# stella-cv/stella_vslam

Hardware: NVIDIA H100
Metric: frames/sec (ORB+match+local BA) @1920x1080, 2000 kpts (higher is better)
Workload: dtype u8

## Files before the change

stella_vslam_b200/csrc/common.cuh:

```cuda
#pragma once

#include <cuda_runtime.h>

#include <cstdarg>
#include <cstdio>
#include <cstring>
#include <string>

#include <nvtx3/nvToolsExt.h>

#include "../../include/b200vslam.h"

namespace b200 {

void set_error(const char* fmt, ...);
int cuda_fail(cudaError_t e, const char* what, const char* file, int line);

#define B200_CUDA(expr)                                                          \
    do {                                                                         \
        cudaError_t _e = (expr);                                                 \
        if (_e != cudaSuccess) return ::b200::cuda_fail(_e, #expr, __FILE__, __LINE__); \
    } while (0)

template <typename T>
__host__ __device__ constexpr T ceil_div(T a, T b) {
    return (a + b - 1) / b;
}
template <typename T>
__host__ __device__ constexpr T round_up(T a, T b) {
    return ceil_div(a, b) * b;
}

struct NvtxRange {
    explicit NvtxRange(const char* name) { nvtxRangePushA(name); }
    ~NvtxRange() { nvtxRangePop(); }
    NvtxRange(const NvtxRange&) = delete;
    NvtxRange& operator=(const NvtxRange&) = delete;
};
#define B200_CAT2(a, b) a##b
#define B200_CAT(a, b) B200_CAT2(a, b)
#define B200_RANGE(name) ::b200::NvtxRange B200_CAT(b200_nvtx_range_, __LINE__)(name)

int require_device(int device);

struct StagingArena;

namespace lba {
int staging(b200_lba_t h, size_t dev_bytes, size_t host_bytes, cudaStream_t* stream, StagingArena** arena);
}

}
```

stella_vslam_b200/csrc/match_kernels.cu:

```cuda
#include <algorithm>
#include <climits>
#include <cmath>
#include <cstddef>
#include <type_traits>
#include <new>
#include <cstring>
#include <vector>

#include "common.cuh"
#include "essential_ransac.cuh"
#include "staging.cuh"
#include "track_chain.cuh"
#include "triangulate.cuh"

namespace b200 {
namespace match {

constexpr int kTopK = 8;
constexpr int kListRowAlign = 64;
constexpr unsigned kInfKey = 0xFFFFFFFFu;
constexpr unsigned kSentinelIdx = 0x3FFFFFu;
constexpr int kThrLow = 50;
constexpr int kMaxDist = 256;

__device__ __forceinline__ unsigned make_key(unsigned dist, unsigned idx) { return (dist << 22) | idx; }
__device__ __forceinline__ unsigned key_dist(unsigned key) { return key >> 22; }
__device__ __forceinline__ unsigned key_idx(unsigned key) { return key & 0x3FFFFFu; }

__device__ __forceinline__ float angle_diff(float a1, float a2) {
    float ret = __fsub_rn(a1, a2);
    if (ret <= -180.0f) ret = __fadd_rn(ret, 360.0f);
    if (ret > 180.0f) ret = __fsub_rn(ret, 360.0f);
    return ret;
}
__device__ __forceinline__ bool orientation_rejects(float a1, float a2) {
    return fabsf(angle_diff(a1, a2)) > 30.0f;
}

__device__ __forceinline__ unsigned hamming256(const uint4& a0, const uint4& a1, const uint4& b0, const uint4& b1) {
    return __popc(a0.x ^ b0.x) + __popc(a0.y ^ b0.y) + __popc(a0.z ^ b0.z) + __popc(a0.w ^ b0.w) + __popc(a1.x ^ b1.x)
           + __popc(a1.y ^ b1.y) + __popc(a1.z ^ b1.z) + __popc(a1.w ^ b1.w);
}

__global__ void __launch_bounds__(256) hamming_matrix_kernel(const uint4* __restrict__ d1, int n1, const uint4* __restrict__ d2, int n2,
                                                             unsigned short* __restrict__ out) {
    __shared__ uint4 s2[64 * 2];
    const int j0 = blockIdx.x * 64, i = blockIdx.y * blockDim.x + threadIdx.x;
    for (int t = threadIdx.x; t < 128; t += blockDim.x) s2[t] = (j0 + t / 2 < n2) ? d2[(size_t)j0 * 2 + t] : make_uint4(0, 0, 0, 0);
    __syncthreads();
    if (i >= n1) return;
    const uint4 a0 = d1[(size_t)i * 2], a1 = d1[(size_t)i * 2 + 1];
    for (int j = 0; j < 64 && j0 + j < n2; ++j) out[(size_t)i * n2 + j0 + j] = (unsigned short)hamming256(a0, a1, s2[2 * j], s2[2 * j + 1]);
}

struct Side {
    const uint4* desc;
    const unsigned char* angle;
    long long angle_stride;
    const int* off;
    const int* cnt;
};
__device__ __forceinline__ float side_angle(const Side& s, int i) {
    return *reinterpret_cast<const float*>(s.angle + (long long)i * s.angle_stride);
}

constexpr int kTcRows = 128;
constexpr int kTcChunk = 128;
constexpr int kTcThreads = 256;
constexpr int kTcTileBytes = 128 * 256;
struct TcSmem {
    unsigned char a[kTcTileBytes];
    unsigned char b[2][kTcTileBytes];
    uint2 lut[256];
    float ang[2][kTcChunk];
};
__device__ __forceinline__ unsigned long long gmma_desc_k_major(unsigned smem_addr, unsigned lbo_bytes, unsigned sbo_bytes) {
    return (unsigned long long)((smem_addr >> 4) & 0x3FFFu) | ((unsigned long long)((lbo_bytes >> 4) & 0x3FFFu) << 16)
           | ((unsigned long long)((sbo_bytes >> 4) & 0x3FFFu) << 32);
}
__device__ __forceinline__ void wgmma_s8_m64n128k32(unsigned (&d)[64], unsigned long long da, unsigned long long db, unsigned accumulate) {
    asm volatile(
        "{\n\t.reg .pred p;\n\t"
        "setp.ne.b32 p, %66, 0;\n\t"
        "wgmma.mma_async.sync.aligned.m64n128k32.s32.s8.s8 {%0, %1, %2, %3, %4, %5, %6, %7, %8, %9, %10, %11, %12, %13, %14, %15, %16, %17, "
        "%18, %19, %20, %21, %22, %23, %24, %25, %26, %27, %28, %29, %30, %31, %32, %33, %34, %35, %36, %37, %38, %39, %40, %41, %42, %43, %44, "
        "%45, %46, %47, %48, %49, %50, %51, %52, %53, %54, %55, %56, %57, %58, %59, %60, %61, %62, %63}, %64, %65, p;\n\t}"
        : "+r"(d[0]), "+r"(d[1]), "+r"(d[2]), "+r"(d[3]), "+r"(d[4]), "+r"(d[5]), "+r"(d[6]), "+r"(d[7]), "+r"(d[8]), "+r"(d[9]), "+r"(d[10]),
          "+r"(d[11]), "+r"(d[12]), "+r"(d[13]), "+r"(d[14]), "+r"(d[15]), "+r"(d[16]), "+r"(d[17]), "+r"(d[18]), "+r"(d[19]), "+r"(d[20]),
          "+r"(d[21]), "+r"(d[22]), "+r"(d[23]), "+r"(d[24]), "+r"(d[25]), "+r"(d[26]), "+r"(d[27]), "+r"(d[28]), "+r"(d[29]), "+r"(d[30]),
          "+r"(d[31]), "+r"(d[32]), "+r"(d[33]), "+r"(d[34]), "+r"(d[35]), "+r"(d[36]), "+r"(d[37]), "+r"(d[38]), "+r"(d[39]), "+r"(d[40]),
          "+r"(d[41]), "+r"(d[42]), "+r"(d[43]), "+r"(d[44]), "+r"(d[45]), "+r"(d[46]), "+r"(d[47]), "+r"(d[48]), "+r"(d[49]), "+r"(d[50]),
          "+r"(d[51]), "+r"(d[52]), "+r"(d[53]), "+r"(d[54]), "+r"(d[55]), "+r"(d[56]), "+r"(d[57]), "+r"(d[58]), "+r"(d[59]), "+r"(d[60]),
          "+r"(d[61]), "+r"(d[62]), "+r"(d[63])
        : "l"(da), "l"(db), "r"(accumulate)
        : "memory");
}
__device__ __forceinline__ void wgmma_fence_operands(unsigned (&d)[64]) {
#pragma unroll
    for (int i = 0; i < 64; ++i) asm volatile("" : "+r"(d[i])::"memory");
}
__device__ __forceinline__ void tc_expand_half(unsigned char* tile, const uint2* lut, int r, int c0, uint4 bits) {
    unsigned char* dst = tile + (r >> 3) * 128 + (r & 7) * 16;
    const unsigned w[4] = {bits.x, bits.y, bits.z, bits.w};
#pragma unroll
    for (int i = 0; i < 8; ++i) {
        const unsigned hw = (w[i >> 1] >> (16 * (i & 1))) & 0xFFFFu;
        const uint2 lo = lut[hw & 0xFFu], hi = lut[hw >> 8];
        *reinterpret_cast<uint4*>(dst + (c0 + i) * 2048) = make_uint4(lo.x, lo.y, hi.x, hi.y);
    }
}
__device__ __forceinline__ void tc_zero_half(unsigned char* tile, int r, int c0) {
    unsigned char* dst = tile + (r >> 3) * 128 + (r & 7) * 16;
#pragma unroll
    for (int i = 0; i < 8; ++i) *reinterpret_cast<uint4*>(dst + (c0 + i) * 2048) = make_uint4(0, 0, 0, 0);
}
__device__ __forceinline__ void insert_key(unsigned (&top)[kTopK], unsigned key) {
    top[kTopK - 1] = key;
#pragma unroll
    for (int k = kTopK - 1; k > 0; --k) {
        if (top[k] < top[k - 1]) {
            const unsigned t = top[k];
            top[k] = top[k - 1];
            top[k - 1] = t;
        }
    }
}

__global__ void __launch_bounds__(kTcThreads, 2) topk_tc_kernel(Side S1, Side S2, const unsigned char* __restrict__ valid2, int check_orientation,
                                                                unsigned* __restrict__ lists, int list_rows, unsigned cap) {
    extern __shared__ __align__(1024) unsigned char tc_smem_raw[];
    TcSmem& sm = *reinterpret_cast<TcSmem*>(tc_smem_raw);
    const uint4* __restrict__ desc1 = S1.desc;
    const uint4* __restrict__ desc2 = S2.desc;
    const int p = blockIdx.y;
    const int b1 = S1.off[p], n1 = S1.cnt[p];
    const int b2 = S2.off[p], n2 = S2.cnt[p];
    const int row0 = blockIdx.x * kTcRows;
    if (row0 >= n2) return;
    const int tid = threadIdx.x, lane = tid & 31;
    for (int e = tid; e < 256; e += kTcThreads) {
        unsigned lo = 0, hi = 0;
#pragma unroll
        for (int i = 0; i < 4; ++i) {
            lo |= (((e >> i) & 1) ? 0x01u : 0xFFu) << (8 * i);
            hi |= (((e >> (4 + i)) & 1) ? 0x01u : 0xFFu) << (8 * i);
        }
        sm.lut[e] = make_uint2(lo, hi);
    }
    __syncthreads();
    const int rtid = tid & 127, half = tid >> 7;
    if (row0 + rtid < n2) tc_expand_half(sm.a, sm.lut, rtid, 8 * half, desc2[(size_t)(b2 + row0 + rtid) * 2 + half]);
    else tc_zero_half(sm.a, rtid, 8 * half);
    const int r_lo = 64 * half + 16 * ((tid >> 5) & 3) + (lane >> 2);
    bool active[2];
    float qa[2];
    unsigned thr[2], top[2][kTopK];
#pragma unroll
    for (int h = 0; h < 2; ++h) {
        const int row = row0 + r_lo + 8 * h;
        active[h] = row < n2 && (!valid2 || valid2[b2 + row]);
        qa[h] = active[h] ? side_angle(S2, b2 + row) : 0.f;
        thr[h] = active[h] ? make_key(cap + 1u, 0u) : 0u;
#pragma unroll
        for (int k = 0; k < kTopK; ++k) top[h][k] = kInfKey;
    }
    const unsigned a_addr = (unsigned)__cvta_generic_to_shared(sm.a) + (unsigned)(half * 8 * 128);
    const unsigned b_addr[2] = {(unsigned)__cvta_generic_to_shared(sm.b[0]), (unsigned)__cvta_generic_to_shared(sm.b[1])};
    const int n_chunks = (n1 + kTcChunk - 1) / kTcChunk;
    uint4 nb = make_uint4(0, 0, 0, 0);
    float nang = 0.f;
    auto fetch = [&](int j) {
        if (j < n1) {
            nb = desc1[(size_t)(b1 + j) * 2 + half];
            if (half == 0) nang = side_angle(S1, b1 + j);
        }
    };
    auto stage = [&](int c) {
        const int j = c * kTcChunk + rtid;
        if (j < n1) {
            tc_expand_half(sm.b[c & 1], sm.lut, rtid, 8 * half, nb);
            if (half == 0) sm.ang[c & 1][rtid] = nang;
        } else {
            tc_zero_half(sm.b[c & 1], rtid, 8 * half);
        }
        fetch(j + kTcChunk);
    };
    fetch(rtid);
    if (n_chunks > 0) stage(0);
    asm volatile("fence.proxy.async.shared::cta;" ::: "memory");
    __syncthreads();
    unsigned acc[64];
#pragma unroll
    for (int i = 0; i < 64; ++i) acc[i] = 0u;
    for (int c = 0; c < n_chunks; ++c) {
        const int buf = c & 1, c0 = c * kTcChunk;
        wgmma_fence_operands(acc);
        asm volatile("wgmma.fence.sync.aligned;" ::: "memory");
#pragma unroll
        for (int ks = 0; ks < 8; ++ks)
            wgmma_s8_m64n128k32(acc, gmma_desc_k_major(a_addr + ks * 4096, 2048, 128), gmma_desc_k_major(b_addr[buf] + ks * 4096, 2048, 128),
                                ks > 0 ? 1u : 0u);
        asm volatile("wgmma.commit_group.sync.aligned;" ::: "memory");
        if (c + 1 < n_chunks) {
            stage(c + 1);
            asm volatile("fence.proxy.async.shared::cta;" ::: "memory");
        }
        asm volatile("wgmma.wait_group.sync.aligned 0;" ::: "memory");
        wgmma_fence_operands(acc);
        const unsigned kbase = (256u << 21) + (unsigned)c0;
        auto scan = [&](auto full_chunk) {
#pragma unroll
            for (int i = 0; i < kTcChunk / 8; ++i) {
                const int col = 8 * i + 2 * (lane & 3);
                unsigned key[2][2];
#pragma unroll
                for (int h = 0; h < 2; ++h)
#pragma unroll
                    for (int u = 0; u < 2; ++u) {
                        key[h][u] = (unsigned)((int)acc[4 * i + 2 * h + u] * -(1 << 21)) + (kbase + (unsigned)(col + u));
                        if (!decltype(full_chunk)::value && c0 + col + u >= n1) key[h][u] = kInfKey;
                    }
                const bool hit = min(key[0][0], key[0][1]) < thr[0] || min(key[1][0], key[1][1]) < thr[1];
                if (__any_sync(0xFFFFFFFFu, hit)) {
#pragma unroll
                    for (int h = 0; h < 2; ++h)
#pragma unroll
                        for (int u = 0; u < 2; ++u) {
                            if (key[h][u] < thr[h]) {
                                if (check_orientation && orientation_rejects(sm.ang[buf][col + u], qa[h])) continue;
                                insert_key(top[h], key[h][u]);
                                thr[h] = min(thr[h], top[h][kTopK - 1]);
                            }
                        }
                }
            }
        };
        if (c0 + kTcChunk <= n1) scan(std::true_type{});
        else scan(std::false_type{});
        __syncthreads();
    }
    unsigned* park = reinterpret_cast<unsigned*>(sm.b[0]);
#pragma unroll
    for (int h = 0; h < 2; ++h)
#pragma unroll
        for (int k = 0; k < kTopK; ++k) park[((r_lo + 8 * h) * 4 + (lane & 3)) * kTopK + k] = top[h][k];
    __syncthreads();
    if (tid < kTcRows) {
        unsigned t[kTopK];
#pragma unroll
        for (int k = 0; k < kTopK; ++k) t[k] = park[tid * 4 * kTopK + k];
        for (int q = 1; q < 4; ++q) {
#pragma unroll
            for (int k2 = 0; k2 < kTopK; ++k2) {
                const unsigned key = park[(tid * 4 + q) * kTopK + k2];
                if (key < t[kTopK - 1]) insert_key(t, key);
            }
        }
#pragma unroll
        for (int k = 0; k < kTopK; ++k)
            if (t[k] == kInfKey && cap < (unsigned)kMaxDist) t[k] = make_key(cap + 1u, kSentinelIdx);
        if (row0 + tid < n2) {
            unsigned* o = lists + ((size_t)p * list_rows + row0 + tid) * kTopK;
#pragma unroll
            for (int k = 0; k < kTopK; ++k) o[k] = t[k];
        }
    }
}

__device__ __forceinline__ unsigned warp_min(unsigned v) {
#pragma unroll
    for (int s = 16; s > 0; s >>= 1) v = min(v, __shfl_xor_sync(0xFFFFFFFFu, v, s));
    return v;
}

__device__ void exact_row(const uint4* desc1, const unsigned char* angle1, long long angle_stride, int n1, const volatile unsigned* taken,
                          uint4 q0, uint4 q1, float qa, int check_orientation, int lane, unsigned* best_key, unsigned* second_dist) {
    unsigned k1 = kInfKey, k2 = kInfKey;
    for (int i0 = lane; i0 < n1; i0 += 128) {
        uint4 a0[4], a1[4];
        float ang[4];
#pragma unroll
        for (int u = 0; u < 4; ++u) {
            const int i = min(i0 + 32 * u, n1 - 1);
            a0[u] = desc1[(size_t)i * 2];
            a1[u] = desc1[(size_t)i * 2 + 1];
            ang[u] = *reinterpret_cast<const float*>(angle1 + (long long)i * angle_stride);
        }
#pragma unroll
        for (int u = 0; u < 4; ++u) {
            const int i = i0 + 32 * u;
            if (i >= n1) continue;
            if ((taken[i >> 5] >> (i & 31)) & 1u) continue;
            if (check_orientation && orientation_rejects(ang[u], qa)) continue;
            const unsigned key = make_key(hamming256(q0, q1, a0[u], a1[u]), (unsigned)i);
            if (key < k1) {
                k2 = k1;
                k1 = key;
            } else if (key < k2) {
                k2 = key;
            }
        }
    }
    const unsigned b = warp_min(k1);
    const unsigned mine = (k1 == b) ? k2 : k1;
    const unsigned s = warp_min(mine);
    *best_key = b;
    *second_dist = (s == kInfKey) ? (unsigned)kMaxDist : key_dist(s);
}

__device__ __forceinline__ int decide_row(const unsigned (&keys)[kTopK], bool full, unsigned tail_dist, const volatile unsigned* taken, float lowe_ratio,
                                          unsigned* best) {
    unsigned best_key = kInfKey, second_dist = kMaxDist;
    int n_live = 0;
#pragma unroll
    for (int k = 0; k < kTopK; ++k) {
        const unsigned key = keys[k];
        if (key == kInfKey) continue;
        const unsigned i1 = key_idx(key);
        if ((taken[i1 >> 5] >> (i1 & 31)) & 1u) continue;
// ... 1115 lines not shown
        if (!s_removed) continue;
        ++n_removed;
        for (int i = tid; i < K.n; i += kCullThreads) {
            const int l = K.kp_lm[i];
            if (l < 0 || __ldcg(P.live_count + l) == 0) continue;
            const int j = cull_own_obs(P, P.off[l], P.off[l + 1], r);
            P.erased[j] = 1;
            atomicSub(P.live_weight + l, (int)P.weight[j]);
            atomicSub(P.live_count + l, 1);
        }
        __syncthreads();
    }
    if (tid == 0) *P.n_removed = n_removed;
}

struct ChainTimer {
    cudaEvent_t ev[7] = {};
    bool timed = false;
    int create() {
        for (cudaEvent_t& e : ev)
            if (!e) B200_CUDA(cudaEventCreate(&e));
        return B200_OK;
    }
    int elapsed(int stage, float* ms) const {
        if (!ms || stage < 0 || stage > 6 || !timed) return B200_ERR_INVALID;
        B200_CUDA(cudaEventElapsedTime(ms, ev[stage == 6 ? 0 : stage], ev[stage == 6 ? 6 : stage + 1]));
        return B200_OK;
    }
    void destroy() {
        for (cudaEvent_t e : ev)
            if (e) cudaEventDestroy(e);
    }
};
enum ChainId { kLocalMapChain, kMotionChain, kRobustChain, kBowChain, kChains };

struct Matcher {
    int device = 0;
    cudaStream_t own_stream = nullptr, stream = nullptr;
    cudaStream_t side_stream = nullptr;
    cudaEvent_t ev_topk = nullptr, ev_resolved = nullptr;
    bool async_resolve = false, resolve_pending = false;
    bool timing = false;
    cudaEvent_t ev_t[3] = {nullptr, nullptr, nullptr};
    ChainTimer chain_timers[kChains];
    int join() {
        if (resolve_pending) {
            B200_CUDA(cudaStreamWaitEvent(stream, ev_resolved, 0));
            resolve_pending = false;
        }
        return B200_OK;
    }
    unsigned* d_lists = nullptr;
    size_t lists_cap = 0;
    int* d_matched = nullptr;
    size_t matched_cap = 0;
    unsigned* d_taken = nullptr;
    size_t taken_cap = 0;
    StagingArena arena;

    int grow(void** p, size_t* cap, size_t bytes) {
        if (bytes <= *cap) return B200_OK;
        B200_CUDA(cudaStreamSynchronize(stream));
        if (*p) B200_CUDA(cudaFree(*p));
        *p = nullptr;
        *cap = 0;
        const size_t want = bytes + bytes / 4 + 256;
        B200_CUDA(cudaMalloc(p, want));
        *cap = want;
        return B200_OK;
    }

    int run(cudaStream_t st, int n_problems, const Side& S1, const Side& S2, const void* valid2, int max_n1, int max_n2, float lowe, int check_ori,
            void* pairs, int pairs_stride, void* n_pairs, bool device_call = false) {
        if (n_problems <= 0) return B200_OK;
        if (max_n1 >= (1 << 22) - 1) {
            set_error("brute-force matcher supports < 4194304 keypoints per frame");
            return B200_ERR_INVALID;
        }
        int rc;
        if ((rc = join())) return rc;
        max_n1 = std::max(max_n1, 1);
        if (pairs_stride < max_n1) {
            set_error("pairs_stride %d is smaller than the largest frame (%d keypoints)", pairs_stride, max_n1);
            return B200_ERR_CAPACITY;
        }
        const int taken_words = ceil_div(max_n1, 32);
        const int list_rows = std::max(1, ceil_div(max_n2, kListRowAlign)) * kListRowAlign;
        if ((rc = grow((void**)&d_lists, &lists_cap, sizeof(unsigned) * kTopK * (size_t)list_rows * n_problems))) return rc;
        if ((rc = grow((void**)&d_matched, &matched_cap, sizeof(int) * (size_t)max_n1 * n_problems))) return rc;
        if ((rc = grow((void**)&d_taken, &taken_cap, sizeof(unsigned) * (size_t)taken_words * n_problems))) return rc;
        if (timing) B200_CUDA(cudaEventRecord(ev_t[0], st));
        const float need = lowe > 0.f ? std::ceil((float)kThrLow / lowe) + 1.f : (float)kMaxDist;
        const unsigned cap = (unsigned)std::min((float)kMaxDist, std::max((float)kThrLow, need));
        B200_CUDA(cudaFuncSetAttribute(topk_tc_kernel, cudaFuncAttributeMaxDynamicSharedMemorySize, (int)sizeof(TcSmem) + 1024));
        topk_tc_kernel<<<dim3(ceil_div(std::max(max_n2, 1), kTcRows), n_problems), kTcThreads, sizeof(TcSmem) + 1024, st>>>(
            S1, S2, (const unsigned char*)valid2, check_ori, d_lists, list_rows, cap);
        if (timing) B200_CUDA(cudaEventRecord(ev_t[1], st));
        const size_t state_bytes = sizeof(unsigned) * ((size_t)taken_words + 2 * (size_t)max_n1);
        const size_t stage_bytes = sizeof(unsigned) * 9 * (size_t)max_n1;
        const int use_smem = (state_bytes + stage_bytes <= 200 * 1024) ? 2 : (state_bytes <= 200 * 1024 ? 1 : 0);
        const size_t rs_bytes = use_smem == 2 ? state_bytes + stage_bytes : state_bytes;
        if (use_smem && rs_bytes > 48 * 1024)
            B200_CUDA(cudaFuncSetAttribute(resolve_kernel, cudaFuncAttributeMaxDynamicSharedMemorySize, (int)rs_bytes));
        cudaStream_t rs = st;
        if (async_resolve && device_call) {
            B200_CUDA(cudaEventRecord(ev_topk, st));
            B200_CUDA(cudaStreamWaitEvent(side_stream, ev_topk, 0));
            rs = side_stream;
        }
        resolve_kernel<<<n_problems, 32, use_smem ? rs_bytes : 0, rs>>>(S1, S2, (const unsigned char*)valid2, d_lists, lowe, check_ori, d_matched,
                                                                        d_taken, taken_words, list_rows, max_n1, pairs_stride, (int*)pairs,
                                                                        (int*)n_pairs, use_smem);
        B200_CUDA(cudaGetLastError());
        if (timing) B200_CUDA(cudaEventRecord(ev_t[2], rs));
        if (rs != st) {
            B200_CUDA(cudaEventRecord(ev_resolved, side_stream));
            resolve_pending = true;
        }
        return B200_OK;
    }
};

template <class Dev = GuidedDev>
static int guided_resolve_smem(const char* who, int n, size_t* bytes) {
    *bytes = (size_t)std::max(n, 1) * 6 + 16;
    if (*bytes > 200 * 1024) {
        set_error("%s: %d keypoints per frame exceed the on-chip occupancy table", who, n);
        return B200_ERR_CAPACITY;
    }
    if (*bytes > 48 * 1024)
        B200_CUDA(cudaFuncSetAttribute(guided_resolve_kernel<Dev>, cudaFuncAttributeMaxDynamicSharedMemorySize, (int)*bytes));
    return B200_OK;
}

}
}

struct b200_matcher_s {
    b200::match::Matcher m;
};

namespace b200 {
namespace chain {
using match::GuidedDev;

static bool search_params_valid(const b200_track_params_t& p) {
    return p.grid_cols > 0 && p.grid_rows > 0 && (long long)p.grid_cols * p.grid_rows <= (1 << 20) && p.img_bounds[1] > p.img_bounds[0]
           && p.img_bounds[3] > p.img_bounds[2] && p.max_candidates >= 0;
}
// ... 245 lines not shown
    sh.k4 = p.cam.k4; sh.distortion = p.cam.distortion;
    sh.cols = p.cam.cols; sh.rows = p.cam.rows;
    sh.fxb = p.focal_x_baseline;
    sh.min_x = p.img_bounds[0]; sh.max_x = p.img_bounds[1]; sh.min_y = p.img_bounds[2]; sh.max_y = p.img_bounds[3];
    sh.ray_cos_thr = p.ray_cos_thr;
    sh.log_scale_factor = p.log_scale_factor;
    sh.margin = p.margin;
    sh.delta = p.monocular ? std::sqrt(5.99146f) : std::sqrt(7.81473f);
    sh.num_levels = p.num_levels;
    for (unsigned l = 0; l < 32; ++l) {
        sh.scale_factors[l] = p.scale_factors[std::min(l, p.num_levels - 1)];
        sh.inv_level_sigma_sq[l] = p.inv_level_sigma_sq[std::min(l, p.num_levels - 1)];
    }
    sh.monocular = p.monocular ? 1 : 0;
    sh.true_baseline = true_baseline;
    return sh;
}
}
}

using b200::match::Side;

extern "C" {

int b200_matcher_create(int device, b200_matcher_t* out) {
    if (!out) return B200_ERR_INVALID;
    int rc = b200::require_device(device);
    if (rc) return rc;
    b200_matcher_s* h = new (std::nothrow) b200_matcher_s();
    if (!h) return B200_ERR_INVALID;
    h->m.device = device;
    cudaError_t e = cudaStreamCreateWithFlags(&h->m.own_stream, cudaStreamNonBlocking);
    if (e == cudaSuccess) e = cudaStreamCreateWithFlags(&h->m.side_stream, cudaStreamNonBlocking);
    if (e == cudaSuccess) e = cudaEventCreateWithFlags(&h->m.ev_topk, cudaEventDisableTiming);
    if (e == cudaSuccess) e = cudaEventCreateWithFlags(&h->m.ev_resolved, cudaEventDisableTiming);
    for (int i = 0; i < 3 && e == cudaSuccess; ++i) e = cudaEventCreate(&h->m.ev_t[i]);
    if (e != cudaSuccess) {
        delete h;
        return b200::cuda_fail(e, "stream creation", __FILE__, __LINE__);
    }
    h->m.stream = h->m.own_stream;
    *out = h;
    return B200_OK;
}

int b200_matcher_destroy(b200_matcher_t h) {
    if (!h) return B200_OK;
    cudaSetDevice(h->m.device);
    cudaStreamSynchronize(h->m.stream);
    if (h->m.side_stream) cudaStreamSynchronize(h->m.side_stream);
    cudaFree(h->m.d_lists);
    cudaFree(h->m.d_matched);
    cudaFree(h->m.d_taken);
    h->m.arena.release();
    for (int i = 0; i < 3; ++i)
        if (h->m.ev_t[i]) cudaEventDestroy(h->m.ev_t[i]);
    for (b200::match::ChainTimer& t : h->m.chain_timers) t.destroy();
    if (h->m.ev_topk) cudaEventDestroy(h->m.ev_topk);
    if (h->m.ev_resolved) cudaEventDestroy(h->m.ev_resolved);
    if (h->m.side_stream) cudaStreamDestroy(h->m.side_stream);
    if (h->m.own_stream) cudaStreamDestroy(h->m.own_stream);
    delete h;
    return B200_OK;
}

int b200_matcher_set_async_resolve(b200_matcher_t h, int enable) {
    if (!h) return B200_ERR_INVALID;
    int rc = h->m.join();
    if (rc) return rc;
    h->m.async_resolve = enable != 0;
    return B200_OK;
}

int b200_matcher_enable_timing(b200_matcher_t h, int enable) {
    if (!h) return B200_ERR_INVALID;
    h->m.timing = enable != 0;
    return B200_OK;
}

int b200_matcher_stage_ms(b200_matcher_t h, int stage, float* ms) {
    if (!h || !ms || stage < 0 || stage > 1) return B200_ERR_INVALID;
    B200_CUDA(cudaEventSynchronize(h->m.ev_t[stage + 1]));
    B200_CUDA(cudaEventElapsedTime(ms, h->m.ev_t[stage], h->m.ev_t[stage + 1]));
    return B200_OK;
}

int b200_matcher_join(b200_matcher_t h) {
    if (!h) return B200_ERR_INVALID;
    return h->m.join();
}

int b200_matcher_set_stream(b200_matcher_t h, void* stream, int use_own) {
    if (!h) return B200_ERR_INVALID;
    B200_CUDA(cudaStreamSynchronize(h->m.stream));
    if (h->m.side_stream) B200_CUDA(cudaStreamSynchronize(h->m.side_stream));
    h->m.resolve_pending = false;
    h->m.stream = use_own ? h->m.own_stream : (cudaStream_t)stream;
    return B200_OK;
}

int b200_matcher_sync(b200_matcher_t h) {
    if (!h) return B200_ERR_INVALID;
    if (h->m.resolve_pending) {
        B200_CUDA(cudaStreamSynchronize(h->m.side_stream));
        h->m.resolve_pending = false;
    }
// ... 1404 lines not shown
    B200_CUDA(cudaGetLastError());
    B200_CUDA(A.download(in_bytes, out_end, st));
    B200_CUDA(cudaStreamSynchronize(st));
    for (int p = 0; p < n_problems; ++p) {
        b200_cull_problem_t& P = problems[p];
        const int* o = A.host<const int>(lay[p].out);
        P.n_removed = o[0];
        for (int r = 0; r < P.n_covisibilities; ++r) {
            b200_cull_keyframe_t& K = P.covisibilities[r];
            K.n_valid = o[1 + 4 * r];
            K.n_redundant = o[2 + 4 * r];
            K.skipped = o[3 + 4 * r];
            K.removed = o[4 + 4 * r];
        }
        P.status = B200_OK;
    }
    return B200_OK;
}

int b200_match_cross_check(const int32_t* idx2_in_1, int n1, const int32_t* idx1_in_2, int n2, int32_t* mutual_out, int32_t* n_mutual) {
    if (n1 < 0 || n2 < 0 || (n1 > 0 && (!idx2_in_1 || !mutual_out)) || (n2 > 0 && !idx1_in_2)) return B200_ERR_INVALID;
    int n = 0;
    for (int i = 0; i < n1; ++i) {
        const int j = idx2_in_1[i];
        const bool keep = 0 <= j && j < n2 && idx1_in_2[j] == i;
        mutual_out[i] = keep ? j : -1;
        n += keep;
    }
    if (n_mutual) *n_mutual = n;
    return B200_OK;
}

int b200_hamming_matrix(b200_matcher_t h, const uint8_t* desc1, int n1, const uint8_t* desc2, int n2, uint16_t* dist) {
    if (!h || n1 < 0 || n2 < 0) return B200_ERR_INVALID;
    if (n1 == 0 || n2 == 0) return B200_OK;
    if (!desc1 || !desc2 || !dist) return B200_ERR_INVALID;
    auto& m = h->m;
    B200_CUDA(cudaSetDevice(m.device));
    b200::Layout L;
    const size_t o_d1 = L.take((size_t)32 * n1), o_d2 = L.take((size_t)32 * n2), o_out = L.take<uint16_t>((size_t)n1 * n2);
    int rc = m.arena.reserve(L.end, 0, m.stream);
    if (rc) return rc;
    unsigned char* s = m.arena.d;
    B200_CUDA(cudaMemcpyAsync(s + o_d1, desc1, (size_t)32 * n1, cudaMemcpyHostToDevice, m.stream));
    B200_CUDA(cudaMemcpyAsync(s + o_d2, desc2, (size_t)32 * n2, cudaMemcpyHostToDevice, m.stream));
    b200::match::hamming_matrix_kernel<<<dim3(b200::ceil_div(n2, 64), b200::ceil_div(n1, 256)), 256, 0, m.stream>>>(
        (const uint4*)(s + o_d1), n1, (const uint4*)(s + o_d2), n2, (unsigned short*)(s + o_out));
    B200_CUDA(cudaGetLastError());
    B200_CUDA(cudaMemcpyAsync(dist, s + o_out, sizeof(uint16_t) * (size_t)n1 * n2, cudaMemcpyDeviceToHost, m.stream));
    B200_CUDA(cudaStreamSynchronize(m.stream));
    return B200_OK;
}

}

namespace b200 {
namespace mapping {

using match::PairsDev;
using tri::TriKfDev;

struct TriProblemDev {
    int k1, k2;
    float cos_thr, ratio_factor;
    int begin;
};

__global__ void __launch_bounds__(256) triangulate_pairs_kernel(const TriKfDev* __restrict__ kfs, const TriProblemDev* __restrict__ ps, int n_problems,
                                                                int total, const int2* __restrict__ matches, double* __restrict__ pos_w,
                                                                unsigned char* __restrict__ ok, int* __restrict__ unconverged) {
    const int t = blockIdx.x * blockDim.x + threadIdx.x;
    if (t >= total) return;
    int lo = 0, hi = n_problems - 1;
    while (lo < hi) {
        const int mid = (lo + hi + 1) >> 1;
        if (ps[mid].begin <= t) lo = mid;
        else hi = mid - 1;
    }
    const TriProblemDev& P = ps[lo];
    const int2 m = matches[t];
    double p[3];
    const int r = tri::two_view_triangulate(kfs[P.k1], kfs[P.k2], m.x, m.y, P.cos_thr, P.ratio_factor, p);
    if (r < 0) atomicAdd(unconverged, 1);
    pos_w[3 * (size_t)t] = p[0];
    pos_w[3 * (size_t)t + 1] = p[1];
    pos_w[3 * (size_t)t + 2] = p[2];
    ok[t] = r == 1;
}

struct ChainKfDev {
    int cur;
    int n_nb;
    int nb_begin;
    int* n_created_rank;
    int* n_created;
    int* created_rank;
    int2* created_idx;
    double* created_pos;
};

constexpr int kClaimThreads = 256;

__global__ void __launch_bounds__(kClaimThreads) landmark_claim_kernel(const TriKfDev* __restrict__ kfs, const float2* __restrict__ nb_consts, const ChainKfDev* __restrict__ ks,
                                                                       const PairsDev* __restrict__ pairs, int n_kf, int rank,
                                                                       int* __restrict__ unconverged) {
    __shared__ int warp_total[kClaimThreads / 32];
// ... 451 lines not shown
```

stella_vslam_b200/csrc/orb_kernels.cu:

```cuda
#include <cuda.h>

#include <algorithm>
#include <cmath>
#include <new>
#include <vector>

#include "camera_model.cuh"
#include "common.cuh"
#include "staging.cuh"
#include "track_chain.cuh"
#include "util_trig.cuh"

namespace b200 {
namespace orb {

constexpr int kMaxLevels = 16;
constexpr int kBorder = 19;
constexpr int kCell = 64;
constexpr int kOverlap = 6;
constexpr int kTileMax = kCell + kOverlap;
constexpr int kTilePitch = 80;

struct LevelGeom {
    int w, h, pitch;
    unsigned long long offset;
    float sf;
    int nx, ny;
    double delta_x, delta_y;
    int grid_base;
    int ncols;
    float size;
    int tab_x, tab_y;
};

struct Geom {
    int num_levels;
    int grid_cells;
    int ini_thr, min_thr;
    LevelGeom lv[kMaxLevels];
};

struct CellDesc {
    unsigned short level, i, j, min_x, min_y, w, h, pad;
};

struct RawKp {
    short x, y;
    unsigned char m;
    unsigned char level;
    unsigned short pad;
};

struct ResizeTap {
    short ofs, w0, w1, pad;
};

struct Images {
    const unsigned char* img0;
    unsigned long long pitch0, fstride0;
    unsigned char* pyr;
    unsigned long long pyr_fstride;
};

__device__ __forceinline__ const unsigned char* level_ptr(const Images& im, const Geom& g, int level, int frame, int* pitch) {
    if (level == 0) {
        *pitch = (int)im.pitch0;
        return im.img0 + (size_t)frame * im.fstride0;
    }
    *pitch = g.lv[level].pitch;
    return im.pyr + (size_t)frame * im.pyr_fstride + g.lv[level].offset;
}

struct TmapSet {
    CUtensorMap m[kMaxLevels];
};

__device__ __forceinline__ unsigned smem_u32(const void* p) { return (unsigned)__cvta_generic_to_shared(p); }

__device__ __forceinline__ void mbar_init(unsigned long long* bar, unsigned count) {
    asm volatile("mbarrier.init.shared::cta.b64 [%0], %1;" ::"r"(smem_u32(bar)), "r"(count));
    asm volatile("fence.mbarrier_init.release.cluster;" ::: "memory");
}
__device__ __forceinline__ void mbar_expect_tx(unsigned long long* bar, unsigned bytes) {
    asm volatile("mbarrier.arrive.expect_tx.shared::cta.b64 _, [%0], %1;" ::"r"(smem_u32(bar)), "r"(bytes) : "memory");
}
__device__ __forceinline__ void mbar_wait(unsigned long long* bar, unsigned parity) {
    asm volatile(
        "{\n\t.reg .pred p;\n\t"
        "WAIT_%=:\n\t"
        "mbarrier.try_wait.parity.shared::cta.b64 p, [%0], %1;\n\t"
        "@p bra DONE_%=;\n\t"
        "bra WAIT_%=;\n\t"
        "DONE_%=:\n\t}" ::"r"(smem_u32(bar)),
        "r"(parity)
        : "memory");
}
__device__ __forceinline__ void tma_load_3d(void* smem_dst, const CUtensorMap* tmap, int x, int y, int z, unsigned long long* bar) {
    asm volatile("cp.async.bulk.tensor.3d.shared::cluster.global.mbarrier::complete_tx::bytes [%0], [%1, {%2, %3, %4}], [%5];" ::"r"(
                     smem_u32(smem_dst)),
                 "l"(reinterpret_cast<unsigned long long>(tmap)), "r"(x), "r"(y), "r"(z), "r"(smem_u32(bar))
                 : "memory");
}

constexpr int kRzRows = 8;

__global__ void __launch_bounds__(128) resize_kernel(const __grid_constant__ Geom g, Images im, const ResizeTap* __restrict__ taps, int level) {
    const LevelGeom& L = g.lv[level];
    const int frame = blockIdx.z;
    int spitch;
    const unsigned char* src = level_ptr(im, g, level - 1, frame, &spitch);
    unsigned char* dst = im.pyr + (size_t)frame * im.pyr_fstride + L.offset;
    const int sw = g.lv[level - 1].w, sh = g.lv[level - 1].h;
    const int dxq = (blockIdx.x * blockDim.x + threadIdx.x) * 4;
    const int dy0 = blockIdx.y * kRzRows;
    if (dxq >= L.pitch) return;
    const int n_valid = min(4, L.w - dxq);
    const unsigned store_mask = n_valid >= 4 ? 0xFFFFFFFFu : (n_valid <= 0 ? 0u : ((1u << (8 * n_valid)) - 1u));
    int ofs[4], ofs1[4];
    unsigned w01[4];
#pragma unroll
    for (int k = 0; k < 4; ++k) {
        const ResizeTap t = taps[L.tab_x + min(dxq + k, L.w - 1)];
        ofs[k] = t.ofs;
        ofs1[k] = min((int)t.ofs + 1, sw - 1);
        w01[k] = ((unsigned)t.w0 & 0xFFFFu) | ((unsigned)t.w1 << 16);
    }
    int rowA = -1, rowB = -1;
    unsigned hA[4] = {0, 0, 0, 0}, hB[4] = {0, 0, 0, 0};
    auto hrow = [&](int sy, unsigned (&h)[4]) {
        const unsigned char* r = src + (size_t)sy * spitch;
#pragma unroll
        for (int k = 0; k < 4; ++k) h[k] = __dp2a_lo(w01[k], (unsigned)r[ofs[k]] | ((unsigned)r[ofs1[k]] << 8), 0u) >> 4;
    };
    const int dy_end = min(dy0 + kRzRows, L.h);
    unsigned char* drow = dst + (size_t)dy0 * L.pitch + dxq;
    for (int dy = dy0; dy < dy_end; ++dy, drow += L.pitch) {
        const ResizeTap ty = taps[L.tab_y + dy];
        const int s0 = min(max((int)ty.ofs, 0), sh - 1), s1 = min(max((int)ty.ofs + 1, 0), sh - 1);
        if (s0 != rowA) {
            if (s0 == rowB) {
#pragma unroll
                for (int k = 0; k < 4; ++k) hA[k] = hB[k];
            } else {
                hrow(s0, hA);
            }
            rowA = s0;
        }
        if (s1 != rowB) {
            if (s1 == rowA) {
// ... 1958 lines not shown
```

Before: 10260.

## Pre-expand B descriptors once and stream them via bulk-async copies in top-k

Adds a separate kernel that expands each problem's S1 descriptors into the ±1 int8 tile layout (plus angles) once in global memory. The top-k tensor-core kernel then loads these pre-expanded chunks with mbarrier-tracked bulk async copies into a double-buffered ring, so expansion is no longer repeated by every row block. Orientation gating moves into the branch-free scan, and a warp-quad threshold tightening runs after each chunk. This costs extra global memory and bandwidth for the expanded tiles (about 32KB per 128 descriptors) plus one more kernel launch, and adds optional phase-profiling instrumentation.

```diff
diff --git a/stella_vslam_b200/csrc/common.cuh b/stella_vslam_b200/csrc/common.cuh
--- a/stella_vslam_b200/csrc/common.cuh
+++ b/stella_vslam_b200/csrc/common.cuh
@@ -45,6 +45,27 @@
 
 struct StagingArena;
 
+__device__ __forceinline__ unsigned smem_u32(const void* p) { return (unsigned)__cvta_generic_to_shared(p); }
+
+__device__ __forceinline__ void mbar_init(unsigned long long* bar, unsigned count) {
+    asm volatile("mbarrier.init.shared::cta.b64 [%0], %1;" ::"r"(smem_u32(bar)), "r"(count));
+    asm volatile("fence.mbarrier_init.release.cluster;" ::: "memory");
+}
+__device__ __forceinline__ void mbar_expect_tx(unsigned long long* bar, unsigned bytes) {
+    asm volatile("mbarrier.arrive.expect_tx.shared::cta.b64 _, [%0], %1;" ::"r"(smem_u32(bar)), "r"(bytes) : "memory");
+}
+__device__ __forceinline__ void mbar_wait(unsigned long long* bar, unsigned parity) {
+    asm volatile(
+        "{\n\t.reg .pred p;\n\t"
+        "WAIT_%=:\n\t"
+        "mbarrier.try_wait.parity.shared::cta.b64 p, [%0], %1;\n\t"
+        "@p bra DONE_%=;\n\t"
+        "bra WAIT_%=;\n\t"
+        "DONE_%=:\n\t}" ::"r"(smem_u32(bar)),
+        "r"(parity)
+        : "memory");
+}
+
 namespace lba {
 int staging(b200_lba_t h, size_t dev_bytes, size_t host_bytes, cudaStream_t* stream, StagingArena** arena);
 }
diff --git a/stella_vslam_b200/csrc/match_kernels.cu b/stella_vslam_b200/csrc/match_kernels.cu
--- a/stella_vslam_b200/csrc/match_kernels.cu
+++ b/stella_vslam_b200/csrc/match_kernels.cu
@@ -68,11 +68,17 @@
 constexpr int kTcChunk = 128;
 constexpr int kTcThreads = 256;
 constexpr int kTcTileBytes = 128 * 256;
+struct TcChunk {
+    unsigned char b[kTcTileBytes];
+    float ang[kTcChunk];
+};
+constexpr int kTcChunkBytes = (int)sizeof(TcChunk);
+static_assert(kTcChunkBytes % 128 == 0, "B tiles of the ring stay 128-byte aligned");
 struct TcSmem {
     unsigned char a[kTcTileBytes];
-    unsigned char b[2][kTcTileBytes];
+    TcChunk chunk[2];
     uint2 lut[256];
-    float ang[2][kTcChunk];
+    unsigned long long full[2];
 };
 __device__ __forceinline__ unsigned long long gmma_desc_k_major(unsigned smem_addr, unsigned lbo_bytes, unsigned sbo_bytes) {
     return (unsigned long long)((smem_addr >> 4) & 0x3FFFu) | ((unsigned long long)((lbo_bytes >> 4) & 0x3FFFu) << 16)
@@ -109,6 +115,15 @@
         *reinterpret_cast<uint4*>(dst + (c0 + i) * 2048) = make_uint4(lo.x, lo.y, hi.x, hi.y);
     }
 }
+__device__ __forceinline__ uint2 tc_lut_entry(int e) {
+    unsigned lo = 0, hi = 0;
+#pragma unroll
+    for (int i = 0; i < 4; ++i) {
+        lo |= (((e >> i) & 1) ? 0x01u : 0xFFu) << (8 * i);
+        hi |= (((e >> (4 + i)) & 1) ? 0x01u : 0xFFu) << (8 * i);
+    }
+    return make_uint2(lo, hi);
+}
 __device__ __forceinline__ void tc_zero_half(unsigned char* tile, int r, int c0) {
     unsigned char* dst = tile + (r >> 3) * 128 + (r & 7) * 16;
 #pragma unroll
@@ -126,28 +141,58 @@
     }
 }
 
-__global__ void __launch_bounds__(kTcThreads, 2) topk_tc_kernel(Side S1, Side S2, const unsigned char* __restrict__ valid2, int check_orientation,
+#ifdef B200_TOPK_PHASES
+enum { kPhWarpChunks, kPhIssueStage, kPhWait, kPhScan, kPhInsert, kPhHits, kPhInserts, kPhSync, kPhMerge, kPhRows, kPhGated, kPhCount };
+constexpr int kPhHistBins = 66;
+__device__ unsigned long long g_topk_phase[kPhCount + kPhHistBins];
+#define TOPK_PH(...) __VA_ARGS__
+#else
+#define TOPK_PH(...)
+#endif
+
+__global__ void __launch_bounds__(256) topk_expand_kernel(Side S1, unsigned char* __restrict__ bexp, int chunk_stride) {
+    __shared__ uint2 lut[256];
+    const int p = blockIdx.y, c = blockIdx.x;
+    const int b1 = S1.off[p], n1 = S1.cnt[p];
+    if (c * kTcChunk >= n1) return;
+    const int tid = threadIdx.x, r = tid & 127, half = tid >> 7, j = c * kTcChunk + r;
+    lut[tid] = tc_lut_entry(tid);
+    __syncthreads();
+    TcChunk* dst = reinterpret_cast<TcChunk*>(bexp + ((size_t)p * chunk_stride + c) * kTcChunkBytes);
+    if (j < n1) tc_expand_half(dst->b, lut, r, 8 * half, S1.desc[(size_t)(b1 + j) * 2 + half]);
+    else tc_zero_half(dst->b, r, 8 * half);
+    if (half == 0) dst->ang[r] = j < n1 ? side_angle(S1, b1 + j) : 0.f;
+}
+
+__global__ void __launch_bounds__(kTcThreads, 2) topk_tc_kernel(Side S1, Side S2, const unsigned char* __restrict__ bexp, int chunk_stride,
+                                                                const unsigned char* __restrict__ valid2, int check_orientation,
                                                                 unsigned* __restrict__ lists, int list_rows, unsigned cap) {
     extern __shared__ __align__(1024) unsigned char tc_smem_raw[];
     TcSmem& sm = *reinterpret_cast<TcSmem*>(tc_smem_raw);
-    const uint4* __restrict__ desc1 = S1.desc;
     const uint4* __restrict__ desc2 = S2.desc;
     const int p = blockIdx.y;
-    const int b1 = S1.off[p], n1 = S1.cnt[p];
+    const int n1 = S1.cnt[p];
     const int b2 = S2.off[p], n2 = S2.cnt[p];
     const int row0 = blockIdx.x * kTcRows;
     if (row0 >= n2) return;
     const int tid = threadIdx.x, lane = tid & 31;
-    for (int e = tid; e < 256; e += kTcThreads) {
-        unsigned lo = 0, hi = 0;
-#pragma unroll
-        for (int i = 0; i < 4; ++i) {
-            lo |= (((e >> i) & 1) ? 0x01u : 0xFFu) << (8 * i);
-            hi |= (((e >> (4 + i)) & 1) ? 0x01u : 0xFFu) << (8 * i);
-        }
-        sm.lut[e] = make_uint2(lo, hi);
+    for (int e = tid; e < 256; e += kTcThreads) sm.lut[e] = tc_lut_entry(e);
+    if (tid == 0) {
+        mbar_init(&sm.full[0], 1);
+        mbar_init(&sm.full[1], 1);
     }
     __syncthreads();
+    const int n_chunks = min((n1 + kTcChunk - 1) / kTcChunk, chunk_stride);
+    const unsigned char* bsrc = bexp + (size_t)p * chunk_stride * kTcChunkBytes;
+    auto load = [&](int c) {
+        unsigned long long* bar = &sm.full[c & 1];
+        mbar_expect_tx(bar, (unsigned)kTcChunkBytes);
+        asm volatile("cp.async.bulk.shared::cluster.global.mbarrier::complete_tx::bytes [%0], [%1], %2, [%3];" ::"r"(smem_u32(&sm.chunk[c & 1])),
+                     "l"(bsrc + (size_t)c * kTcChunkBytes), "r"((unsigned)kTcChunkBytes), "r"(smem_u32(bar))
+                     : "memory");
+    };
+    if (tid == 0)
+        for (int c = 0; c < min(2, n_chunks); ++c) load(c);
     const int rtid = tid & 127, half = tid >> 7;
     if (row0 + rtid < n2) tc_expand_half(sm.a, sm.lut, rtid, 8 * half, desc2[(size_t)(b2 + row0 + rtid) * 2 + half]);
     else tc_zero_half(sm.a, rtid, 8 * half);
@@ -165,35 +210,17 @@
         for (int k = 0; k < kTopK; ++k) top[h][k] = kInfKey;
     }
     const unsigned a_addr = (unsigned)__cvta_generic_to_shared(sm.a) + (unsigned)(half * 8 * 128);
-    const unsigned b_addr[2] = {(unsigned)__cvta_generic_to_shared(sm.b[0]), (unsigned)__cvta_generic_to_shared(sm.b[1])};
-    const int n_chunks = (n1 + kTcChunk - 1) / kTcChunk;
-    uint4 nb = make_uint4(0, 0, 0, 0);
-    float nang = 0.f;
-    auto fetch = [&](int j) {
-        if (j < n1) {
-            nb = desc1[(size_t)(b1 + j) * 2 + half];
-            if (half == 0) nang = side_angle(S1, b1 + j);
-        }
-    };
-    auto stage = [&](int c) {
-        const int j = c * kTcChunk + rtid;
-        if (j < n1) {
-            tc_expand_half(sm.b[c & 1], sm.lut, rtid, 8 * half, nb);
-            if (half == 0) sm.ang[c & 1][rtid] = nang;
-        } else {
-            tc_zero_half(sm.b[c & 1], rtid, 8 * half);
-        }
-        fetch(j + kTcChunk);
-    };
-    fetch(rtid);
-    if (n_chunks > 0) stage(0);
+    const unsigned b_addr[2] = {smem_u32(sm.chunk[0].b), smem_u32(sm.chunk[1].b)};
     asm volatile("fence.proxy.async.shared::cta;" ::: "memory");
     __syncthreads();
     unsigned acc[64];
 #pragma unroll
     for (int i = 0; i < 64; ++i) acc[i] = 0u;
+    TOPK_PH(unsigned long long ph[kPhCount] = {}; unsigned n_pass[2] = {0u, 0u}, n_gated[2] = {0u, 0u}; long long t0 = clock64(); long long t1 = t0;)
     for (int c = 0; c < n_chunks; ++c) {
         const int buf = c & 1, c0 = c * kTcChunk;
+        TOPK_PH(t0 = clock64(); ph[kPhWarpChunks] += 1;)
+        mbar_wait(&sm.full[buf], (unsigned)(c >> 1) & 1u);
         wgmma_fence_operands(acc);
         asm volatile("wgmma.fence.sync.aligned;" ::: "memory");
 #pragma unroll
@@ -201,17 +228,16 @@
             wgmma_s8_m64n128k32(acc, gmma_desc_k_major(a_addr + ks * 4096, 2048, 128), gmma_desc_k_major(b_addr[buf] + ks * 4096, 2048, 128),
                                 ks > 0 ? 1u : 0u);
         asm volatile("wgmma.commit_group.sync.aligned;" ::: "memory");
-        if (c + 1 < n_chunks) {
-            stage(c + 1);
-            asm volatile("fence.proxy.async.shared::cta;" ::: "memory");
-        }
+        TOPK_PH(t1 = clock64(); ph[kPhIssueStage] += t1 - t0; t0 = t1;)
         asm volatile("wgmma.wait_group.sync.aligned 0;" ::: "memory");
         wgmma_fence_operands(acc);
+        TOPK_PH(t1 = clock64(); ph[kPhWait] += t1 - t0; t0 = t1;)
         const unsigned kbase = (256u << 21) + (unsigned)c0;
-        auto scan = [&](auto full_chunk) {
+        auto scan = [&](auto full_chunk, auto gate) {
 #pragma unroll
             for (int i = 0; i < kTcChunk / 8; ++i) {
                 const int col = 8 * i + 2 * (lane & 3);
+                const float2 ang = decltype(gate)::value ? *reinterpret_cast<const float2*>(&sm.chunk[buf].ang[col]) : make_float2(0.f, 0.f);
                 unsigned key[2][2];
 #pragma unroll
                 for (int h = 0; h < 2; ++h)
@@ -219,27 +245,48 @@
                     for (int u = 0; u < 2; ++u) {
                         key[h][u] = (unsigned)((int)acc[4 * i + 2 * h + u] * -(1 << 21)) + (kbase + (unsigned)(col + u));
                         if (!decltype(full_chunk)::value && c0 + col + u >= n1) key[h][u] = kInfKey;
+                        TOPK_PH(n_pass[h] += active[h] && key[h][u] < make_key(cap + 1u, 0u);)
+                        if (decltype(gate)::value && orientation_rejects(u ? ang.y : ang.x, qa[h])) key[h][u] = kInfKey;
+                        TOPK_PH(n_gated[h] += active[h] && key[h][u] < make_key(cap + 1u, 0u);)
                     }
                 const bool hit = min(key[0][0], key[0][1]) < thr[0] || min(key[1][0], key[1][1]) < thr[1];
                 if (__any_sync(0xFFFFFFFFu, hit)) {
+                    TOPK_PH(const long long ti = clock64(); ph[kPhHits] += 1;)
 #pragma unroll
                     for (int h = 0; h < 2; ++h)
 #pragma unroll
                         for (int u = 0; u < 2; ++u) {
                             if (key[h][u] < thr[h]) {
-                                if (check_orientation && orientation_rejects(sm.ang[buf][col + u], qa[h])) continue;
                                 insert_key(top[h], key[h][u]);
                                 thr[h] = min(thr[h], top[h][kTopK - 1]);
+                                TOPK_PH(ph[kPhInserts] += 1;)
                             }
                         }
+                    TOPK_PH(ph[kPhInsert] += clock64() - ti;)
                 }
             }
         };
-        if (c0 + kTcChunk <= n1) scan(std::true_type{});
-        else scan(std::false_type{});
+        const bool full = c0 + kTcChunk <= n1;
+        if (check_orientation) full ? scan(std::true_type{}, std::true_type{}) : scan(std::false_type{}, std::true_type{});
+        else full ? scan(std::true_type{}, std::false_type{}) : scan(std::false_type{}, std::false_type{});
+#pragma unroll
+        for (int h = 0; h < 2; ++h) {
+            unsigned b7 = min(top[h][7], __shfl_xor_sync(0xFFFFFFFFu, top[h][7], 1));
+            b7 = min(b7, __shfl_xor_sync(0xFFFFFFFFu, b7, 2));
+            unsigned b1 = max(top[h][1], __shfl_xor_sync(0xFFFFFFFFu, top[h][1], 1));
+            b1 = max(b1, __shfl_xor_sync(0xFFFFFFFFu, b1, 2));
+            const unsigned o3 = __shfl_xor_sync(0xFFFFFFFFu, top[h][3], 1);
+            const unsigned lo = min(top[h][3], o3), hi = max(top[h][3], o3);
+            const unsigned b3 = min(max(lo, __shfl_xor_sync(0xFFFFFFFFu, lo, 2)), min(hi, __shfl_xor_sync(0xFFFFFFFFu, hi, 2)));
+            thr[h] = min(thr[h], min(b7, min(b1, b3)));
+        }
+        TOPK_PH(t1 = clock64(); ph[kPhScan] += t1 - t0; t0 = t1;)
         __syncthreads();
-    }
-    unsigned* park = reinterpret_cast<unsigned*>(sm.b[0]);
+        TOPK_PH(ph[kPhSync] += clock64() - t0;)
+        if (tid == 0 && c + 2 < n_chunks) load(c + 2);
+    }
+    TOPK_PH(t0 = clock64();)
+    unsigned* park = reinterpret_cast<unsigned*>(sm.chunk[0].b);
 #pragma unroll
     for (int h = 0; h < 2; ++h)
 #pragma unroll
@@ -265,6 +312,30 @@
             for (int k = 0; k < kTopK; ++k) o[k] = t[k];
         }
     }
+#ifdef B200_TOPK_PHASES
+    __syncthreads();
+    ph[kPhMerge] += clock64() - t0;
+    for (int h = 0; h < 2; ++h) {
+        n_pass[h] += __shfl_xor_sync(0xFFFFFFFFu, n_pass[h], 1);
+        n_pass[h] += __shfl_xor_sync(0xFFFFFFFFu, n_pass[h], 2);
+        if ((lane & 3) == 0 && active[h]) {
+            atomicAdd(&g_topk_phase[kPhCount + min(n_pass[h], (unsigned)kPhHistBins - 1)], 1ull);
+            atomicAdd(&g_topk_phase[kPhRows], 1ull);
+        }
+    }
+    ph[kPhGated] = n_gated[0] + n_gated[1];
+    unsigned long long ins = ph[kPhInserts], gated = ph[kPhGated];
+    for (int s = 16; s > 0; s >>= 1) {
+        ins += __shfl_xor_sync(0xFFFFFFFFu, ins, s);
+        gated += __shfl_xor_sync(0xFFFFFFFFu, gated, s);
+    }
+    if (lane == 0) {
+        ph[kPhInserts] = ins;
+        ph[kPhGated] = gated;
+        for (int k = 0; k < kPhCount; ++k)
+            if (k != kPhRows) atomicAdd(&g_topk_phase[k], ph[k]);
+    }
+#endif
 }
 
 __device__ __forceinline__ unsigned warp_min(unsigned v) {
@@ -1486,6 +1557,8 @@
     }
     unsigned* d_lists = nullptr;
     size_t lists_cap = 0;
+    unsigned char* d_bexp = nullptr;
+    size_t bexp_cap = 0;
     int* d_matched = nullptr;
     size_t matched_cap = 0;
     unsigned* d_taken = nullptr;
@@ -1523,12 +1596,15 @@
         if ((rc = grow((void**)&d_lists, &lists_cap, sizeof(unsigned) * kTopK * (size_t)list_rows * n_problems))) return rc;
         if ((rc = grow((void**)&d_matched, &matched_cap, sizeof(int) * (size_t)max_n1 * n_problems))) return rc;
         if ((rc = grow((void**)&d_taken, &taken_cap, sizeof(unsigned) * (size_t)taken_words * n_problems))) return rc;
+        const int chunk_stride = ceil_div(max_n1, kTcChunk);
+        if ((rc = grow((void**)&d_bexp, &bexp_cap, (size_t)kTcChunkBytes * chunk_stride * n_problems))) return rc;
         if (timing) B200_CUDA(cudaEventRecord(ev_t[0], st));
         const float need = lowe > 0.f ? std::ceil((float)kThrLow / lowe) + 1.f : (float)kMaxDist;
         const unsigned cap = (unsigned)std::min((float)kMaxDist, std::max((float)kThrLow, need));
+        topk_expand_kernel<<<dim3(chunk_stride, n_problems), 256, 0, st>>>(S1, d_bexp, chunk_stride);
         B200_CUDA(cudaFuncSetAttribute(topk_tc_kernel, cudaFuncAttributeMaxDynamicSharedMemorySize, (int)sizeof(TcSmem) + 1024));
         topk_tc_kernel<<<dim3(ceil_div(std::max(max_n2, 1), kTcRows), n_problems), kTcThreads, sizeof(TcSmem) + 1024, st>>>(
-            S1, S2, (const unsigned char*)valid2, check_ori, d_lists, list_rows, cap);
+            S1, S2, d_bexp, chunk_stride, (const unsigned char*)valid2, check_ori, d_lists, list_rows, cap);
         if (timing) B200_CUDA(cudaEventRecord(ev_t[1], st));
         const size_t state_bytes = sizeof(unsigned) * ((size_t)taken_words + 2 * (size_t)max_n1);
         const size_t stage_bytes = sizeof(unsigned) * 9 * (size_t)max_n1;
@@ -1880,6 +1956,7 @@
     cudaFree(h->m.d_lists);
     cudaFree(h->m.d_matched);
     cudaFree(h->m.d_taken);
+    cudaFree(h->m.d_bexp);
     h->m.arena.release();
     for (int i = 0; i < 3; ++i)
         if (h->m.ev_t[i]) cudaEventDestroy(h->m.ev_t[i]);
@@ -3390,6 +3467,17 @@
     return B200_OK;
 }
 
+#ifdef B200_TOPK_PHASES
+int b200_topk_phase_counters(unsigned long long* out, int n) {
+    using namespace b200::match;
+    if (n < kPhCount + kPhHistBins) return B200_ERR_INVALID;
+    B200_CUDA(cudaDeviceSynchronize());
+    B200_CUDA(cudaMemcpyFromSymbol(out, g_topk_phase, sizeof(g_topk_phase)));
+    static const unsigned long long zero[kPhCount + kPhHistBins] = {};
+    B200_CUDA(cudaMemcpyToSymbol(g_topk_phase, zero, sizeof(zero)));
+    return B200_OK;
+}
+#endif
 }
 
 namespace b200 {
diff --git a/stella_vslam_b200/csrc/orb_kernels.cu b/stella_vslam_b200/csrc/orb_kernels.cu
--- a/stella_vslam_b200/csrc/orb_kernels.cu
+++ b/stella_vslam_b200/csrc/orb_kernels.cu
@@ -75,26 +75,6 @@
     CUtensorMap m[kMaxLevels];
 };
 
-__device__ __forceinline__ unsigned smem_u32(const void* p) { return (unsigned)__cvta_generic_to_shared(p); }
-
-__device__ __forceinline__ void mbar_init(unsigned long long* bar, unsigned count) {
-    asm volatile("mbarrier.init.shared::cta.b64 [%0], %1;" ::"r"(smem_u32(bar)), "r"(count));
-    asm volatile("fence.mbarrier_init.release.cluster;" ::: "memory");
-}
-__device__ __forceinline__ void mbar_expect_tx(unsigned long long* bar, unsigned bytes) {
-    asm volatile("mbarrier.arrive.expect_tx.shared::cta.b64 _, [%0], %1;" ::"r"(smem_u32(bar)), "r"(bytes) : "memory");
-}
-__device__ __forceinline__ void mbar_wait(unsigned long long* bar, unsigned parity) {
-    asm volatile(
-        "{\n\t.reg .pred p;\n\t"
-        "WAIT_%=:\n\t"
-        "mbarrier.try_wait.parity.shared::cta.b64 p, [%0], %1;\n\t"
-        "@p bra DONE_%=;\n\t"
-        "bra WAIT_%=;\n\t"
-        "DONE_%=:\n\t}" ::"r"(smem_u32(bar)),
-        "r"(parity)
-        : "memory");
-}
 __device__ __forceinline__ void tma_load_3d(void* smem_dst, const CUtensorMap* tmap, int x, int y, int z, unsigned long long* bar) {
     asm volatile("cp.async.bulk.tensor.3d.shared::cluster.global.mbarrier::complete_tx::bytes [%0], [%1, {%2, %3, %4}], [%5];" ::"r"(
                      smem_u32(smem_dst)),
```

Measured after the change: 10470 (median of 6 runs). +2.0%, better.
